# Gabisanth/MaximumAreaCoverageOptimization.jl

Hardware: AMD Instinct MI355X
Metric: MADS objective evals/sec (N UAVs × M fire cells), 1/2/4/8 MI355X (higher is better)
Workload: dtype f64

## Files before the change

maximumareacoverageoptimization.jl_amd/csrc/k_prep.h:

```cpp
#pragma once

#include <hip/hip_runtime.h>
#include <stdint.h>

#include "predicate.h"
#include "k_common.h"

#pragma clang fp contract(off)

namespace mac {


struct PenArgs {
    const double* rmax;
    const double* prev;
    const double* dlimT;
    const double* dlim;
    double tan_half_fov;
};

__device__ __forceinline__ double pen_threshold(const PenArgs& pa, int i)
{
    if (!pa.prev) return 0.0;
    return pa.dlimT ? pa.dlimT[i] : dlim_threshold(pa.dlim[i]);
}

__device__ __forceinline__ double pen_term(double x2, double y2, double R2, int i, int N,
                                           const PenArgs& pa, double T3)
{
    if (pa.prev) {
        const double x1 = pa.prev[i], y1 = pa.prev[N + i], z1 = pa.prev[2 * N + i] / pa.tan_half_fov;
        const double z2 = R2 / pa.tan_half_fov;
        const double ddx = x1 - x2, ddy = y1 - y2, ddz = z1 - z2;
        const double s = ddx * ddx + ddy * ddy + ddz * ddz;
        if (s > T3) return -1.0;
    }
    return pa.rmax ? __builtin_fabs(R2 - pa.rmax[i]) : 0.0;
}

__host__ __device__ __forceinline__ bool diag_rejects(double v, double b, double p, int q,
                                                      double tan_half_fov, double T3)
{
    bool all = true;
#pragma unroll
    for (int sg = 0; sg < 2; ++sg) {
        const double c = sg == 0 ? v + b : v - b;
        double d;
        if (q < 2) {
            d = p - c;
        } else {
            const double z1 = p / tan_half_fov, z2 = c / tan_half_fov;
            d = z1 - z2;
        }
        const double sq = d * d;
        all = all && sq > T3;
    }
    return all;
}


__host__ __device__ __forceinline__ uint64_t splitmix_at(uint64_t state, uint64_t idx)
{
    uint64_t z = state + idx * 0x9E3779B97F4A7C15ull;
    z = (z ^ (z >> 30)) * 0xBF58476D1CE4E5B9ull;
    z = (z ^ (z >> 27)) * 0x94D049BB133111EBull;
    return z ^ (z >> 31);
}

__host__ __device__ __forceinline__ double splitmix_uniform_at(uint64_t state, uint64_t idx)
{
    return (double)(splitmix_at(state, idx) >> 11) * (1.0 / 9007199254740992.0);
}

__host__ __device__ __forceinline__ double ltmads_entry(uint64_t state, int64_t n, int64_t b,
                                                        int64_t r, int64_t c)
{
    if (r < c) return 0.0;
    if (r == c) return (splitmix_uniform_at(state, (uint64_t)r + 1) < 0.5 ? -1.0 : 1.0) * (double)b;
    const int64_t lo = -b + 1, span = 2 * b - 1;
    const double u = splitmix_uniform_at(state, (uint64_t)(n + 1 + r * (r - 1) / 2 + c));
    return (double)(lo + (int64_t)__builtin_floor(u * (double)span));
}

struct MadsState {
    double f;
    int64_t it;
    int ell;
    int skip;
    unsigned long long feas;
    int64_t skipped;
    int64_t succ;
};

struct CandSrc {
    const double* cands;
    int ldc;
    const uint32_t* keysP;
    const float* keysT;
    int ldk;
    const double* xinc;
    const int* rp;
    const int* cp;
    uint64_t state;
    int64_t b;
    int k0;
    const MadsState* mst;
    const int16_t* ltri;
    double delta;
    int route_five;
    __device__ __forceinline__ bool resolve(bool any_poll = false)
    {
        if (!mst) return true;
        const int e = mst->ell;
        if (e < 0 || (!any_poll && mst->skip)) return false;
        b = (int64_t)1 << e;
        return true;
    }
    __device__ __forceinline__ double entry(int n, int r, int c) const
    {
        if (ltri) return r < c ? 0.0 : delta * (double)ltri[(int64_t)r * (r + 1) / 2 + c];
        return ltmads_entry(state, n, b, r, c);
    }
    __device__ __forceinline__ double get(int kl, int v, int N) const
    {
        if (cands) return cands[(int64_t)kl * ldc + v];
        const int n = 3 * N;
        const int k = kl + k0;
        const int kk = k < n ? k : k - n;
        const double d = entry(n, rp[v], cp[kk]);
        return k < n ? xinc[v] + d : xinc[v] - d;
    }
};

#ifndef MAC_PREP_C
#define MAC_PREP_C 8
#endif
constexpr int kPrepC = MAC_PREP_C;
constexpr int kPrepU = 512;

static_assert(kPrepC % 4 == 0 && 32 % kPrepC == 0 && kPrepC <= 64,
              "MAC_PREP_C must divide 32 and be a multiple of 4");
__host__ __device__ inline int keys_ld(int K) { return (K + 31) & ~31; }

struct PrepArgs {
    CandSrc src;
    int N, K;
    PenArgs pa;
    double penalty;
    double* vp;
    int pair;
    int nchain;
    int skip_failed;
    int4* prec;
    Grid g;
    uint32_t* keysP;
    float* keysT;
    int ldk;
    double4* pd;
    uint8_t* dead8;
    MadsState* mst_w;
    unsigned long long* feas;
    int* lreset;
    int xbase;
};

constexpr int kPrepCX = 6;

constexpr uint32_t kKeyEsc = 0x200u << 22;
__device__ __forceinline__ bool key_int(double v, double b, double lim, int& d)
{
    const double f = v - b;
    if (!(f >= -lim && f <= lim)) return false;
    d = (int)f;
    return (double)d == f && __builtin_bit_cast(uint64_t, b + (double)d) == __builtin_bit_cast(uint64_t, v);
}
__device__ __forceinline__ uint32_t key_pack(int dx, int dy, int dr)
{
    return ((uint32_t)dx & 0x7FFu) | (((uint32_t)dy & 0x7FFu) << 11) | (((uint32_t)dr & 0x3FFu) << 22);
}
__device__ __forceinline__ void key_unpack(uint32_t p, float& x, float& y, float& r)
{
    x = (float)((int)(p << 21) >> 21);
    y = (float)((int)(p << 10) >> 21);
    r = (float)((int)p >> 22);
}

__device__ __forceinline__ bool partial_range(double a, double b, double m, double g0, double invS,
                                              int n, int& lo, int& hi)
{
    const double ulo = (a - g0) * invS;
    const double uhi = (b - g0) * invS;
    const double err = (m + __builtin_fabs(g0)) * invS * 1e-14 + 1e-9;
    const double flo = __builtin_floor(ulo - err);
    const double fhi = __builtin_floor(uhi + err);
    if (!(flo == flo) || !(fhi == fhi)) { lo = 0; hi = n - 1; return true; }
    if (fhi < 0.0 || flo > (double)(n - 1)) return false;
    lo = flo < 0.0 ? 0 : (int)flo;
    hi = fhi > (double)(n - 1) ? n - 1 : (int)fhi;
    return true;
}

__host__ __device__ inline int range_shift(int n)
{
    int s = 0;
    while (((n - 1) >> s) > 0xFFFE) ++s;
    return s;
}
__device__ __forceinline__ uint32_t range_pack(bool any, int lo, int hi, int s)
{
    return any ? (uint32_t)(lo >> s) | ((uint32_t)(hi >> s) << 16) : 0xFFFFu;
}
__device__ __forceinline__ void range_unpack(uint32_t lo16, uint32_t hi16, int s, int n, int& lo, int& hi)
{
    lo = (int)(lo16 << s);
    hi = min((int)(((hi16 + 1) << s) - 1), n - 1);
}

#ifdef MAC_DIAG
__device__ uint64_t g_diag_prep[64 * 16];
#define MAC_PREP_STAMP_T(q, t) if (threadIdx.x == (t) && cw < 64 && (q) < 16) g_diag_prep[16 * cw + (q)] = __builtin_amdgcn_s_memrealtime()
#else
#define MAC_PREP_STAMP_T(q, t)
#endif
#define MAC_PREP_STAMP(q) MAC_PREP_STAMP_T(q, 0)

__device__ __forceinline__ void lds_barrier()
{
    asm volatile("s_waitcnt lgkmcnt(0)\n\ts_barrier" ::: "memory");
}

template <int PC>
struct PrepLds {
    double term[PC][kPrepU + 2];
    int wbad[kPrepU / kWave][PC];
    uint32_t wbadm[kPrepU / kWave];
    int wrej[kPrepU / kWave];
    double dred[kPrepU / kWave][4];
};

template <bool kMat, int PC>
__device__ __forceinline__ void prep_block(const PrepArgs& a, int cw, unsigned char* lds)
{
    constexpr int NC = PC;
    PrepLds<NC>& L = *reinterpret_cast<PrepLds<NC>*>(lds);
    auto& term = L.term;
    auto& wbad = L.wbad;
    auto& wbadm = L.wbadm;
    auto& wrej = L.wrej;
    auto& dred = L.dred;
    const int N = a.N, K = a.K;
    const int u = threadIdx.x, lane = u & (kWave - 1), wid = u / kWave;
    const int k0 = cw * PC;
    const int n3 = 3 * N;
    auto cand = [&](int c) { return a.pair ? (c < 4 ? 4 * cw + c : n3 + 4 * cw + c - 4) : k0 + c; };
    const bool obj = a.vp != nullptr;
    const PenArgs& pa = a.pa;
    MAC_PREP_STAMP(0);
    double acc = 0.0;
    bool bad = false;
    const bool excl = obj && pa.prev && (a.prec || a.pd) && a.skip_failed && N <= kPrepU;
    double dmx = -__builtin_inf(), dmy = -__builtin_inf(), dmr = -__builtin_inf();
    double dml = -__builtin_inf();
    uint32_t dead = 0u;
    for (int ib = 0; ib < N; ib += kPrepU) {
        const int nb = min(kPrepU, N - ib);
        const int i = ib + u;
        const bool iv = u < nb;
        const int ii = min(i, N - 1);
        double v[NC][3];
        if (!kMat && PC == 8 && a.pair) {
#pragma unroll
            for (int c = 0; c < 4; ++c) {
                const int col = 4 * cw + c;
#pragma unroll
                for (int q = 0; q < 3; ++q) {
                    const int vv = q * N + ii;
                    const double d = a.src.entry(n3, a.src.rp[vv], a.src.cp[col]);
                    v[c][q] = a.src.xinc[vv] + d;
                    v[c + 4][q] = a.src.xinc[vv] - d;
                }
            }
        } else {
#pragma unroll
            for (int c = 0; c < NC; ++c) {
                const int k = min(cand(c), K - 1);
#pragma unroll
                for (int q = 0; q < 3; ++q) {
                    if constexpr (kMat) v[c][q] = a.src.cands[(int64_t)k * a.src.ldc + q * N + ii];
                    else v[c][q] = a.src.get(k, q * N + ii, N);
                }
            }
        }
        double base[3] = {0.0, 0.0, 0.0};
        if (a.keysP) {
#pragma unroll
            for (int q = 0; q < 3; ++q) {
                if constexpr (kMat) base[q] = a.src.cands[q * N + ii];
                else base[q] = a.src.get(0, q * N + ii, N);
            }
        }
        if (obj) {
            const double x1 = pa.prev ? pa.prev[ii] : 0.0, y1 = pa.prev ? pa.prev[N + ii] : 0.0;
            const double z1 = pa.prev ? pa.prev[2 * N + ii] / pa.tan_half_fov : 0.0;
            const double rm = pa.rmax ? pa.rmax[ii] : 0.0;
            const double T3 = pen_threshold(pa, ii);
            uint32_t wdead = 0u;
#pragma unroll
            for (int c = 0; c < NC; ++c) {
                const double R2 = v[c][2];
                double t = pa.rmax ? __builtin_fabs(R2 - rm) : 0.0;
                if (pa.prev) {
                    const double z2 = R2 / pa.tan_half_fov;
                    const double ddx = x1 - v[c][0], ddy = y1 - v[c][1], ddz = z1 - z2;
                    const double sq = ddx * ddx + ddy * ddy + ddz * ddz;
                    if (sq > T3) t = -1.0;
                }
                term[c][u] = t;
                const uint64_t neg = __ballot(iv && t < 0.0);
                if (lane == 0) wbad[wid][c] = neg != 0;
                wdead |= (neg != 0 ? 1u : 0u) << c;
            }
            if (lane == 0) wbadm[wid] = wdead;
            if (a.mst_w) {
                bool rej = true;
                if (iv) {
                    const double bb = (double)a.src.b;
                    rej = diag_rejects(a.src.xinc[ii], bb, x1, 0, pa.tan_half_fov, T3) &&
                          diag_rejects(a.src.xinc[N + ii], bb, y1, 1, pa.tan_half_fov, T3) &&
                          diag_rejects(a.src.xinc[2 * N + ii], bb, pa.prev[2 * N + ii], 2, pa.tan_half_fov, T3);
                }
                const uint64_t keep = __ballot(!rej);
                if (lane == 0) wrej[wid] = keep == 0;
            }
            MAC_PREP_STAMP(1 + 3 * (ib / kPrepU));
            lds_barrier();
            if (excl) {
                dead = 0u;
#pragma unroll
                for (int w = 0; w < kPrepU / kWave; ++w) dead |= wbadm[w];
                if (a.mst_w) {
                    bool rej = true;
#pragma unroll
                    for (int w = 0; w < kPrepU / kWave; ++w) rej = rej && wrej[w] != 0;
                    if (cw == 0 && u == 0) a.mst_w->skip = rej ? 1 : 0;
                    if (rej) return;
                }
            }
            if (u < NC) {
#pragma unroll
                for (int w = 0; w < kPrepU / kWave; ++w) bad |= wbad[w][u] != 0;
                if (!bad) {
                    __builtin_amdgcn_s_setprio(3);
                    constexpr int kB = 3;
                    const double2* row2 = reinterpret_cast<const double2*>(&term[u][0]);
                    const int nfull = nb / (2 * kB);
                    auto batch = [&](double2 (&buf)[kB], int bt) {
                        const int at = (bt < nfull ? bt : nfull - 1) * kB;
#pragma unroll
                        for (int j = 0; j < kB; ++j) buf[j] = row2[at + j];
                    };
                    auto add = [&](const double2 (&buf)[kB]) {
#pragma unroll
                        for (int j = 0; j < kB; ++j) {
                            acc += buf[j].x;
                            acc += buf[j].y;
                        }
                    };
                    if (nfull > 0) {
                        double2 A[kB], B[kB];
                        batch(A, 0);
#pragma unroll 1
                        for (int bt = 0; bt < nfull; bt += 2) {
                            batch(B, bt + 1);
                            __builtin_amdgcn_sched_barrier(0);
                            add(A);
                            if (bt + 1 >= nfull) break;
                            batch(A, bt + 2);
                            __builtin_amdgcn_sched_barrier(0);
                            add(B);
                        }
                    }
                    for (int q = nfull * 2 * kB; q < nb; ++q) acc += term[u][q];
                    __builtin_amdgcn_s_setprio(0);
                }
            }
            MAC_PREP_STAMP(2 + 3 * (ib / kPrepU));
        }
        if (a.pd && a.keysP && iv) {
#pragma unroll
            for (int c = 0; c < NC; ++c) {
                const double x = v[c][0], y = v[c][1], r = v[c][2];
                if (cand(c) < K && !((dead >> c) & 1u) && r > 0.0 && __builtin_isfinite(x) &&
                    __builtin_isfinite(y)) {
                    double ex = __builtin_fabs(x - base[0]), ey = __builtin_fabs(y - base[1]), er = r - base[2];
                    double el = base[2] - r;
                    if (!(ex <= kDblMax)) ex = __builtin_inf();
                    if (!(ey <= kDblMax)) ey = __builtin_inf();
                    if (!(er == er)) er = __builtin_inf();
                    if (!(el == el)) el = __builtin_inf();
                    dmx = fmax(dmx, ex);
                    dmy = fmax(dmy, ey);
                    dmr = fmax(dmr, er);
                    dml = fmax(dml, el);
                }
            }
        }
        if (a.pd && ib + kPrepU >= N) {
#pragma unroll
            for (int o = 32; o >= 1; o >>= 1) {
                dmx = fmax(dmx, __shfl_xor(dmx, o, kWave));
                dmy = fmax(dmy, __shfl_xor(dmy, o, kWave));
                dmr = fmax(dmr, __shfl_xor(dmr, o, kWave));
                dml = fmax(dml, __shfl_xor(dml, o, kWave));
            }
            if (lane == 0) {
                dred[wid][0] = dmx;
                dred[wid][1] = dmy;
                dred[wid][2] = dmr;
                dred[wid][3] = dml;
            }
        }
        if ((a.prec || a.keysP) && iv) {
            double xa = __builtin_inf(), xb = -__builtin_inf(), ya = __builtin_inf(), yb = -__builtin_inf();
            double xm = 0.0, ym = 0.0, est = 0.0;
            bool any = false;
#pragma unroll
            for (int c = 0; c < NC; ++c) {
                if (!a.prec) break;
                const double x = v[c][0], y = v[c][1], r = v[c][2];
                if (cand(c) < K && !((dead >> c) & 1u) && r > 0.0 && __builtin_isfinite(x) &&
                    __builtin_isfinite(y)) {
                    any = true;
                    xa = fmin(xa, x - r);
                    xb = fmax(xb, x + r);
                    ya = fmin(ya, y - r);
                    yb = fmax(yb, y + r);
                    xm = fmax(xm, __builtin_fabs(x) + r);
                    ym = fmax(ym, __builtin_fabs(y) + r);
                    const double e = 2.0 * r * a.g.invS + 1.0;
                    est += e * e;
                }
            }
            bool kb = false;
            if (a.keysP) {
                uint32_t pk[NC];
#pragma unroll
                for (int c = 0; c < NC; ++c) {
                    int dx = 0, dy = 0, dr = 0;
                    const bool packs = key_int(v[c][0], base[0], 1023.0, dx) &&
                                       key_int(v[c][1], base[1], 1023.0, dy) &&
                                       key_int(v[c][2], base[2], 511.0, dr);
                    pk[c] = packs ? key_pack(dx, dy, dr) : kKeyEsc;
                    if (!packs) {
#pragma unroll
                        for (int q = 0; q < 3; ++q) {
                            const float f = (float)(v[c][q] - base[q]);
                            kb |= !((dead >> c) & 1u) && __builtin_bit_cast(uint64_t, base[q] + (double)f) != __builtin_bit_cast(uint64_t, v[c][q]);
                            a.keysT[(int64_t)(q * N + i) * a.ldk + cand(c)] = f;
                        }
                    }
                }
                uint32_t* const krow = a.keysP + (int64_t)i * a.ldk;
#pragma unroll
                for (int h = 0; h < PC / 4; ++h)
                    *reinterpret_cast<uint4*>(krow + cand(4 * h)) =
                        make_uint4(pk[4 * h], pk[4 * h + 1], pk[4 * h + 2], pk[4 * h + 3]);
            }
            if (a.prec) {
                int x0 = 0, x1 = -1, y0 = 0, y1 = -1;
                any = any && partial_range(xa, xb, xm, a.g.gx0, a.g.invS, a.g.nTx, x0, x1) &&
                      partial_range(ya, yb, ym, a.g.gy0, a.g.invS, a.g.nTy, y0, y1);
                a.prec[(int64_t)cw * N + i] =
                    make_int4((int)range_pack(any, x0, x1, range_shift(a.g.nTx)),
                              (int)range_pack(any, y0, y1, range_shift(a.g.nTy)),
                              __builtin_bit_cast(int, (float)est), kb ? 1 : 0);
            }
        }
        MAC_PREP_STAMP(3 + 3 * (ib / kPrepU));
        if (obj && ib + kPrepU < N) lds_barrier();
    }
    if (obj && u < NC && cand(u) < K) {
        a.vp[cand(u)] = bad ? __builtin_inf() : acc * a.penalty;
        if (a.dead8) a.dead8[cand(u)] = excl && bad ? 1 : 0;
    }
    if (obj && a.feas && wid == 0) {
        const uint64_t ok = __ballot(u < NC && cand(u) < K && !bad);
        if (lane == 0 && ok) atomicAdd(a.feas, (unsigned long long)__popcll(ok));
    }
    if (a.pd) {
        lds_barrier();
        if (u == 0) {
            double4 m = make_double4(dred[0][0], dred[0][1], dred[0][2], dred[0][3]);
            for (int q = 1; q < kPrepU / kWave; ++q) {
                m.x = fmax(m.x, dred[q][0]);
                m.y = fmax(m.y, dred[q][1]);
                m.z = fmax(m.z, dred[q][2]);
                m.w = fmax(m.w, dred[q][3]);
            }
            a.pd[cw] = m;
        }
    }
}

template <bool kGen>
__device__ __forceinline__ void prep_block_x(const PrepArgs& a, int cw, unsigned char* lds)
{
    constexpr int PC = kPrepCX, NC = kGen ? kPrepCX : kPrepCX + 1, NW = kPrepU / kWave;
    PrepLds<kPrepCX + 1>& L = *reinterpret_cast<PrepLds<kPrepCX + 1>*>(lds);
    auto& term = L.term;
    auto& wbad = L.wbad;
    auto& wbadm = L.wbadm;
    auto& wrej = L.wrej;
    auto& dred = L.dred;
    const int N = a.N, K = a.K;
    const int u = threadIdx.x, lane = u & (kWave - 1), wid = u / kWave;
    const bool fw = wid == NW;
    const int k0 = cw * PC;
    const int n3 = 3 * N;
    auto cand = [&](int c) {
        if constexpr (kGen) return c < 3 ? 3 * cw + c : n3 + 3 * cw + c - 3;
        else return c < PC ? k0 + c : a.xbase + cw;
    };
    const bool obj = a.vp != nullptr;
    const PenArgs& pa = a.pa;
    const bool excl = obj && pa.prev && a.skip_failed;
    const bool iv = !fw && u < N;
    const int ii = min(u, N - 1);
    MAC_PREP_STAMP(0);
    double v[NC][3];
    double base[3] = {0.0, 0.0, 0.0};
    if (!fw) {
        if constexpr (kGen) {
#pragma unroll
            for (int q = 0; q < 3; ++q) {
                const int vv = q * N + ii;
                const int rv = a.src.rp[vv];
                const double xv = a.src.xinc[vv];
#pragma unroll
                for (int c = 0; c < 3; ++c) {
                    const double d = a.src.entry(n3, rv, a.src.cp[3 * cw + c]);
                    v[c][q] = xv + d;
                    v[c + 3][q] = xv - d;
                }
                base[q] = xv + a.src.entry(n3, rv, a.src.cp[0]);
            }
        } else {
#pragma unroll
            for (int c = 0; c < NC; ++c) {
                const int k = min(cand(c), K - 1);
#pragma unroll
                for (int q = 0; q < 3; ++q) v[c][q] = a.src.cands[(int64_t)k * a.src.ldc + q * N + ii];
            }
#pragma unroll
            for (int q = 0; q < 3; ++q) base[q] = a.src.cands[q * N + ii];
        }
        if (obj) {
            const double x1 = pa.prev ? pa.prev[ii] : 0.0, y1 = pa.prev ? pa.prev[N + ii] : 0.0;
            const double z1 = pa.prev ? pa.prev[2 * N + ii] / pa.tan_half_fov : 0.0;
            const double rm = pa.rmax ? pa.rmax[ii] : 0.0;
            const double T3 = pen_threshold(pa, ii);
            uint32_t wdead = 0u;
#pragma unroll
            for (int c = 0; c < NC; ++c) {
                const double R2 = v[c][2];
                double t = pa.rmax ? __builtin_fabs(R2 - rm) : 0.0;
                if (pa.prev) {
                    const double z2 = R2 / pa.tan_half_fov;
                    const double ddx = x1 - v[c][0], ddy = y1 - v[c][1], ddz = z1 - z2;
                    const double sq = ddx * ddx + ddy * ddy + ddz * ddz;
                    if (sq > T3) t = -1.0;
                }
                term[c][u] = t;
                const uint64_t neg = __ballot(iv && t < 0.0);
                if (lane == 0) wbad[wid][c] = neg != 0;
                wdead |= (neg != 0 ? 1u : 0u) << c;
            }
            if (lane == 0) wbadm[wid] = wdead;
            if (a.mst_w) {
                bool rej = true;
                if (iv) {
                    const double bb = (double)a.src.b;
                    rej = diag_rejects(a.src.xinc[ii], bb, x1, 0, pa.tan_half_fov, T3) &&
                          diag_rejects(a.src.xinc[N + ii], bb, y1, 1, pa.tan_half_fov, T3) &&
                          diag_rejects(a.src.xinc[2 * N + ii], bb, pa.prev[2 * N + ii], 2, pa.tan_half_fov, T3);
                }
                const uint64_t keep = __ballot(!rej);
                if (lane == 0) wrej[wid] = keep == 0;
            }
        }
    }
    MAC_PREP_STAMP(1);
    uint32_t dead = 0u;
    if (obj) {
        lds_barrier();
        if (excl) {
#pragma unroll
            for (int w = 0; w < NW; ++w) dead |= wbadm[w];
            if (a.mst_w) {
                bool rej = true;
#pragma unroll
                for (int w = 0; w < NW; ++w) rej = rej && wrej[w] != 0;
                if (cw == 0 && u == 0) a.mst_w->skip = rej ? 1 : 0;
                if (rej) return;
            }
        }
    }
    MAC_PREP_STAMP(2);
    if (fw) {
        bool bad = false;
        double acc = 0.0;
        if (obj && lane < NC) {
#pragma unroll
            for (int w = 0; w < NW; ++w) bad |= wbad[w][lane] != 0;
            if (!bad) {
                constexpr int kB = 6;
                const double2* row2 = reinterpret_cast<const double2*>(&term[lane][0]);
                const int nfull = N / (2 * kB);
                __builtin_amdgcn_s_setprio(3);
                auto batch = [&](double2 (&buf)[kB], int bt) {
                    const int at = (bt < nfull ? bt : nfull - 1) * kB;
#pragma unroll
                    for (int j = 0; j < kB; ++j) buf[j] = row2[at + j];
                };
                auto add = [&](const double2 (&buf)[kB]) {
#pragma unroll
                    for (int j = 0; j < kB; ++j) {
                        acc += buf[j].x;
                        acc += buf[j].y;
                    }
                };
                if (nfull > 0) {
                    double2 A[kB], B[kB];
                    batch(A, 0);
#pragma unroll 1
                    for (int bt = 0; bt < nfull; bt += 2) {
                        batch(B, bt + 1);
                        __builtin_amdgcn_sched_barrier(0);
                        add(A);
                        if (bt + 1 >= nfull) break;
                        batch(A, bt + 2);
                        __builtin_amdgcn_sched_barrier(0);
                        add(B);
                    }
                }
                for (int q = nfull * 2 * kB; q < N; ++q) acc += term[lane][q];
                __builtin_amdgcn_s_setprio(0);
            }
            MAC_PREP_STAMP_T(3, kPrepU);
            if (cand(lane) < K) {
                a.vp[cand(lane)] = bad ? __builtin_inf() : acc * a.penalty;
                if (a.dead8) a.dead8[cand(lane)] = excl && bad ? 1 : 0;
            }
        }
        if (obj && a.feas) {
            const uint64_t ok = __ballot(lane < NC && cand(lane) < K && !bad);
            if (lane == 0 && ok) atomicAdd(a.feas, (unsigned long long)__popcll(ok));
        }
    } else {
        double dmx = -__builtin_inf(), dmy = -__builtin_inf(), dmr = -__builtin_inf(), dml = -__builtin_inf();
        uint32_t pk[NC];
        bool kb = false;
#pragma unroll
        for (int c = 0; c < NC; ++c) {
            const double x = v[c][0], y = v[c][1], r = v[c][2];
            int dx = 0, dy = 0, dr = 0;
            const bool packs = key_int(x, base[0], 1023.0, dx) && key_int(y, base[1], 1023.0, dy) &&
                               key_int(r, base[2], 511.0, dr);
            pk[c] = packs ? key_pack(dx, dy, dr) : kKeyEsc;
            if (!packs && iv && cand(c) < K) {
#pragma unroll
                for (int q = 0; q < 3; ++q) {
                    const float f = (float)(v[c][q] - base[q]);
                    if constexpr (kGen)
                        kb |= !((dead >> c) & 1u) &&
                              __builtin_bit_cast(uint64_t, base[q] + (double)f) != __builtin_bit_cast(uint64_t, v[c][q]);
                    a.keysT[(int64_t)(q * N + u) * a.ldk + cand(c)] = f;
                }
            }
            if (a.pd && iv && cand(c) < K && !((dead >> c) & 1u) && r > 0.0 && __builtin_isfinite(x) &&
                __builtin_isfinite(y)) {
                double ex = __builtin_fabs(x - base[0]), ey = __builtin_fabs(y - base[1]), er = r - base[2];
                double el = base[2] - r;
                if (!(ex <= kDblMax)) ex = __builtin_inf();
                if (!(ey <= kDblMax)) ey = __builtin_inf();
                if (!(er == er)) er = __builtin_inf();
                if (!(el == el)) el = __builtin_inf();
                dmx = fmax(dmx, ex);
                dmy = fmax(dmy, ey);
                dmr = fmax(dmr, er);
                dml = fmax(dml, el);
            }
        }
        if (iv) {
            uint32_t* const krow = a.keysP + (int64_t)u * a.ldk;
            if constexpr (kGen) {
#pragma unroll
                for (int c = 0; c < NC; ++c) krow[cand(c)] = pk[c];
            } else {
                static_assert(PC % 2 == 0, "an even candidate count");
#pragma unroll
                for (int h = 0; h < PC / 2; ++h)
                    *reinterpret_cast<uint2*>(krow + k0 + 2 * h) = make_uint2(pk[2 * h], pk[2 * h + 1]);
                if (cand(PC) < K) krow[cand(PC)] = pk[PC];
            }
        }
        if (kGen && a.prec && iv) {
            double xa = __builtin_inf(), xb = -__builtin_inf(), ya = __builtin_inf(), yb = -__builtin_inf();
            double xm = 0.0, ym = 0.0, est = 0.0;
            bool any = false;
#pragma unroll
            for (int c = 0; c < NC; ++c) {
                const double x = v[c][0], y = v[c][1], r = v[c][2];
                if (cand(c) < K && !((dead >> c) & 1u) && r > 0.0 && __builtin_isfinite(x) &&
                    __builtin_isfinite(y)) {
                    any = true;
                    xa = fmin(xa, x - r);
                    xb = fmax(xb, x + r);
                    ya = fmin(ya, y - r);
                    yb = fmax(yb, y + r);
                    xm = fmax(xm, __builtin_fabs(x) + r);
                    ym = fmax(ym, __builtin_fabs(y) + r);
                    const double e = 2.0 * r * a.g.invS + 1.0;
                    est += e * e;
                }
            }
            int x0 = 0, x1 = -1, y0 = 0, y1 = -1;
            any = any && partial_range(xa, xb, xm, a.g.gx0, a.g.invS, a.g.nTx, x0, x1) &&
                  partial_range(ya, yb, ym, a.g.gy0, a.g.invS, a.g.nTy, y0, y1);
            a.prec[(int64_t)cw * N + u] =
                make_int4((int)range_pack(any, x0, x1, range_shift(a.g.nTx)),
                          (int)range_pack(any, y0, y1, range_shift(a.g.nTy)),
                          __builtin_bit_cast(int, (float)est), kb ? 1 : 0);
        }
        if (a.pd) {
#pragma unroll
            for (int o = 32; o >= 1; o >>= 1) {
                dmx = fmax(dmx, __shfl_xor(dmx, o, kWave));
                dmy = fmax(dmy, __shfl_xor(dmy, o, kWave));
                dmr = fmax(dmr, __shfl_xor(dmr, o, kWave));
                dml = fmax(dml, __shfl_xor(dml, o, kWave));
            }
            if (lane == 0) {
                dred[wid][0] = dmx;
                dred[wid][1] = dmy;
                dred[wid][2] = dmr;
                dred[wid][3] = dml;
            }
        }
    }
    if (a.pd) {
        lds_barrier();
        if (u == 0) {
            double4 m = make_double4(dred[0][0], dred[0][1], dred[0][2], dred[0][3]);
            for (int q = 1; q < NW; ++q) {
                m.x = fmax(m.x, dred[q][0]);
                m.y = fmax(m.y, dred[q][1]);
                m.z = fmax(m.z, dred[q][2]);
                m.w = fmax(m.w, dred[q][3]);
            }
            a.pd[cw] = m;
        }
    }
}

template <int PC, bool kX = false, bool kGen = false>
__device__ __forceinline__ void prep_body(uint64_t* ts, PrepArgs& a)
{
    ts_begin(ts);
    if (a.lreset && blockIdx.x == 0 && threadIdx.x == 0) *a.lreset = 0;
    if (!a.src.resolve(true)) {
        ts_end(ts);
        return;
    }
    const int per = (int)((gridDim.x + 7) / 8), b = (int)blockIdx.x;
    const int cw = (int)(gridDim.x % 8) == 0 ? (b % 8) * per + b / 8 : b;
    __shared__ __attribute__((aligned(16))) unsigned char lds[sizeof(PrepLds<kX ? PC + 1 : PC>)];
    if constexpr (kX) {
        prep_block_x<kGen>(a, cw, lds);
    } else if (a.src.cands) {
        prep_block<true, PC>(a, cw, lds);
    } else {
        prep_block<false, PC>(a, cw, lds);
    }
    ts_end(ts);
}

__global__ __launch_bounds__(kPrepU) __attribute__((amdgpu_waves_per_eu(4))) void prep_kernel(uint64_t* ts, PrepArgs a)
{
    prep_body<kPrepC>(ts, a);
}

template <bool kGen>
__global__ __launch_bounds__(kPrepU + kWave) __attribute__((amdgpu_waves_per_eu(6))) void prep_x_kernel(uint64_t* ts, PrepArgs a)
{
    prep_body<kPrepCX, true, kGen>(ts, a);
}

__global__ void disk_prep_kernel(CandSrc src, int N, int K, DiskRec* __restrict__ disks)
{
    const int64_t t = (int64_t)blockIdx.x * blockDim.x + threadIdx.x;
    if (t >= (int64_t)N * K) return;
    const int k = (int)(t / N), i = (int)(t % N);
    disks[t] = make_disk(src.get(k, i, N), src.get(k, N + i, N), src.get(k, 2 * N + i, N));
}

}
```

Before: 44.17 million.

## Overlap penalty fold and key packing with feasibility checks in prep kernel

Restructures the prep kernel's non-generated path so the rmax penalty terms are written to LDS before the distance check. The fold warp can then sum them while worker warps do the feasibility test and key packing, with global loads ordered by sched_barriers to issue the radius loads first. Key packing for the candidate path now runs before the barrier that waits on failure flags, so packing overlaps the synchronization. In exchange the fold runs even for candidates later marked bad, an extra barrier is added, and the control flow is more complex.

```diff
diff --git a/maximumareacoverageoptimization.jl_amd/csrc/k_prep.h b/maximumareacoverageoptimization.jl_amd/csrc/k_prep.h
--- a/maximumareacoverageoptimization.jl_amd/csrc/k_prep.h
+++ b/maximumareacoverageoptimization.jl_amd/csrc/k_prep.h
@@ -219,8 +219,10 @@
 #ifdef MAC_DIAG
 __device__ uint64_t g_diag_prep[64 * 16];
 #define MAC_PREP_STAMP_T(q, t) if (threadIdx.x == (t) && cw < 64 && (q) < 16) g_diag_prep[16 * cw + (q)] = __builtin_amdgcn_s_memrealtime()
+#define MAC_PREP_STAMP_XY(q) do { asm volatile("s_waitcnt vmcnt(0)" ::: "memory"); MAC_PREP_STAMP_T(q, 0); } while (0)
 #else
 #define MAC_PREP_STAMP_T(q, t)
+#define MAC_PREP_STAMP_XY(q)
 #endif
 #define MAC_PREP_STAMP(q) MAC_PREP_STAMP_T(q, 0)
 
@@ -527,9 +529,84 @@
     const bool iv = !fw && u < N;
     const int ii = min(u, N - 1);
     MAC_PREP_STAMP(0);
-    double v[NC][3];
-    double base[3] = {0.0, 0.0, 0.0};
-    if (!fw) {
+    auto failures = [&](uint32_t& dead) {
+        if (!excl) return false;
+#pragma unroll
+        for (int w = 0; w < NW; ++w) dead |= wbadm[w];
+        if (!a.mst_w) return false;
+        bool rej = true;
+#pragma unroll
+        for (int w = 0; w < NW; ++w) rej = rej && wrej[w] != 0;
+        if (cw == 0 && u == 0) a.mst_w->skip = rej ? 1 : 0;
+        return rej;
+    };
+    auto fold = [&](double& acc) {
+        constexpr int kB = 6;
+        const double2* row2 = reinterpret_cast<const double2*>(&term[lane][0]);
+        const int nfull = N / (2 * kB);
+        __builtin_amdgcn_s_setprio(3);
+        auto batch = [&](double2 (&buf)[kB], int bt) {
+            const int at = (bt < nfull ? bt : nfull - 1) * kB;
+#pragma unroll
+            for (int j = 0; j < kB; ++j) buf[j] = row2[at + j];
+        };
+        auto add = [&](const double2 (&buf)[kB]) {
+#pragma unroll
+            for (int j = 0; j < kB; ++j) {
+                acc += buf[j].x;
+                acc += buf[j].y;
+            }
+        };
+        if (nfull > 0) {
+            double2 A[kB], B[kB];
+            batch(A, 0);
+#pragma unroll 1
+            for (int bt = 0; bt < nfull; bt += 2) {
+                batch(B, bt + 1);
+                __builtin_amdgcn_sched_barrier(0);
+                add(A);
+                if (bt + 1 >= nfull) break;
+                batch(A, bt + 2);
+                __builtin_amdgcn_sched_barrier(0);
+                add(B);
+            }
+        }
+        for (int q = nfull * 2 * kB; q < N; ++q) acc += term[lane][q];
+        __builtin_amdgcn_s_setprio(0);
+    };
+    if (fw) {
+        bool bad = false;
+        double acc = 0.0;
+        if (obj) {
+            const bool mine = lane < NC && cand(lane) < K;
+            if constexpr (!kGen) {
+                lds_barrier();
+                if (mine) fold(acc);
+                MAC_PREP_STAMP_T(3, kPrepU);
+            }
+            lds_barrier();
+            uint32_t dead = 0u;
+            if (failures(dead)) return;
+            if (mine) {
+#pragma unroll
+                for (int w = 0; w < NW; ++w) bad |= wbad[w][lane] != 0;
+                if constexpr (kGen) {
+                    if (!bad) fold(acc);
+                    MAC_PREP_STAMP_T(3, kPrepU);
+                }
+                a.vp[cand(lane)] = bad ? __builtin_inf() : acc * a.penalty;
+                if (a.dead8) a.dead8[cand(lane)] = excl && bad ? 1 : 0;
+            }
+            if (a.feas) {
+                const uint64_t ok = __ballot(mine && !bad);
+                if (lane == 0 && ok) atomicAdd(a.feas, (unsigned long long)__popcll(ok));
+            }
+        }
+    } else {
+        double v[NC][3];
+        double base[3] = {0.0, 0.0, 0.0};
+        double rm = 0.0;
+        double x1 = 0.0, y1 = 0.0, p1 = 0.0, dl = 0.0;
         if constexpr (kGen) {
 #pragma unroll
             for (int q = 0; q < 3; ++q) {
@@ -544,21 +621,46 @@
                 }
                 base[q] = xv + a.src.entry(n3, rv, a.src.cp[0]);
             }
+            if (obj) {
+                if (pa.rmax) rm = pa.rmax[ii];
+                if (pa.prev) {
+                    x1 = pa.prev[ii], y1 = pa.prev[N + ii], p1 = pa.prev[2 * N + ii];
+                    dl = pa.dlimT ? pa.dlimT[ii] : pa.dlim[ii];
+                }
+            }
         } else {
-#pragma unroll
-            for (int c = 0; c < NC; ++c) {
-                const int k = min(cand(c), K - 1);
-#pragma unroll
-                for (int q = 0; q < 3; ++q) v[c][q] = a.src.cands[(int64_t)k * a.src.ldc + q * N + ii];
-            }
+            const double* cp[NC];
+#pragma unroll
+            for (int c = 0; c < NC; ++c) cp[c] = a.src.cands + (int64_t)min(cand(c), K - 1) * a.src.ldc + ii;
+#pragma unroll
+            for (int c = 0; c < NC; ++c) v[c][2] = cp[c][2 * N];
+            const double* const anyp = a.src.cands + ii;
+            rm = *(obj && pa.rmax ? pa.rmax + ii : anyp);
+            __builtin_amdgcn_sched_barrier(0);
 #pragma unroll
             for (int q = 0; q < 3; ++q) base[q] = a.src.cands[q * N + ii];
+            const bool c3 = obj && pa.prev;
+            x1 = *(c3 ? pa.prev + ii : anyp), y1 = *(c3 ? pa.prev + N + ii : anyp);
+            p1 = *(c3 ? pa.prev + 2 * N + ii : anyp);
+            dl = *(!c3 ? anyp : pa.dlimT ? pa.dlimT + ii : pa.dlim + ii);
+            __builtin_amdgcn_sched_barrier(0);
+#pragma unroll
+            for (int c = 0; c < NC; ++c) {
+                v[c][0] = cp[c][0];
+                v[c][1] = cp[c][N];
+                __builtin_amdgcn_sched_barrier(0);
+            }
+            if (obj) {
+#pragma unroll
+                for (int c = 0; c < NC; ++c) term[c][u] = pa.rmax ? __builtin_fabs(v[c][2] - rm) : 0.0;
+                MAC_PREP_STAMP(1);
+                lds_barrier();
+                MAC_PREP_STAMP(2);
+            }
         }
         if (obj) {
-            const double x1 = pa.prev ? pa.prev[ii] : 0.0, y1 = pa.prev ? pa.prev[N + ii] : 0.0;
-            const double z1 = pa.prev ? pa.prev[2 * N + ii] / pa.tan_half_fov : 0.0;
-            const double rm = pa.rmax ? pa.rmax[ii] : 0.0;
-            const double T3 = pen_threshold(pa, ii);
+            const double z1 = pa.prev ? p1 / pa.tan_half_fov : 0.0;
+            const double T3 = !pa.prev ? 0.0 : pa.dlimT ? dl : dlim_threshold(dl);
             uint32_t wdead = 0u;
 #pragma unroll
             for (int c = 0; c < NC; ++c) {
@@ -570,7 +672,7 @@
                     const double sq = ddx * ddx + ddy * ddy + ddz * ddz;
                     if (sq > T3) t = -1.0;
                 }
-                term[c][u] = t;
+                if constexpr (kGen) term[c][u] = t;
                 const uint64_t neg = __ballot(iv && t < 0.0);
                 if (lane == 0) wbad[wid][c] = neg != 0;
                 wdead |= (neg != 0 ? 1u : 0u) << c;
@@ -582,101 +684,64 @@
                     const double bb = (double)a.src.b;
                     rej = diag_rejects(a.src.xinc[ii], bb, x1, 0, pa.tan_half_fov, T3) &&
                           diag_rejects(a.src.xinc[N + ii], bb, y1, 1, pa.tan_half_fov, T3) &&
-                          diag_rejects(a.src.xinc[2 * N + ii], bb, pa.prev[2 * N + ii], 2, pa.tan_half_fov, T3);
+                          diag_rejects(a.src.xinc[2 * N + ii], bb, p1, 2, pa.tan_half_fov, T3);
                 }
                 const uint64_t keep = __ballot(!rej);
                 if (lane == 0) wrej[wid] = keep == 0;
             }
         }
-    }
-    MAC_PREP_STAMP(1);
-    uint32_t dead = 0u;
-    if (obj) {
-        lds_barrier();
-        if (excl) {
-#pragma unroll
-            for (int w = 0; w < NW; ++w) dead |= wbadm[w];
-            if (a.mst_w) {
-                bool rej = true;
-#pragma unroll
-                for (int w = 0; w < NW; ++w) rej = rej && wrej[w] != 0;
-                if (cw == 0 && u == 0) a.mst_w->skip = rej ? 1 : 0;
-                if (rej) return;
-            }
-        }
-    }
-    MAC_PREP_STAMP(2);
-    if (fw) {
-        bool bad = false;
-        double acc = 0.0;
-        if (obj && lane < NC) {
-#pragma unroll
-            for (int w = 0; w < NW; ++w) bad |= wbad[w][lane] != 0;
-            if (!bad) {
-                constexpr int kB = 6;
-                const double2* row2 = reinterpret_cast<const double2*>(&term[lane][0]);
-                const int nfull = N / (2 * kB);
-                __builtin_amdgcn_s_setprio(3);
-                auto batch = [&](double2 (&buf)[kB], int bt) {
-                    const int at = (bt < nfull ? bt : nfull - 1) * kB;
-#pragma unroll
-                    for (int j = 0; j < kB; ++j) buf[j] = row2[at + j];
-                };
-                auto add = [&](const double2 (&buf)[kB]) {
-#pragma unroll
-                    for (int j = 0; j < kB; ++j) {
-                        acc += buf[j].x;
-                        acc += buf[j].y;
-                    }
-                };
-                if (nfull > 0) {
-                    double2 A[kB], B[kB];
-                    batch(A, 0);
-#pragma unroll 1
-                    for (int bt = 0; bt < nfull; bt += 2) {
-                        batch(B, bt + 1);
-                        __builtin_amdgcn_sched_barrier(0);
-                        add(A);
-                        if (bt + 1 >= nfull) break;
-                        batch(A, bt + 2);
-                        __builtin_amdgcn_sched_barrier(0);
-                        add(B);
-                    }
-                }
-                for (int q = nfull * 2 * kB; q < N; ++q) acc += term[lane][q];
-                __builtin_amdgcn_s_setprio(0);
-            }
-            MAC_PREP_STAMP_T(3, kPrepU);
-            if (cand(lane) < K) {
-                a.vp[cand(lane)] = bad ? __builtin_inf() : acc * a.penalty;
-                if (a.dead8) a.dead8[cand(lane)] = excl && bad ? 1 : 0;
-            }
-        }
-        if (obj && a.feas) {
-            const uint64_t ok = __ballot(lane < NC && cand(lane) < K && !bad);
-            if (lane == 0 && ok) atomicAdd(a.feas, (unsigned long long)__popcll(ok));
-        }
-    } else {
+        uint32_t dead = 0u;
+        bool kb = false;
+        auto escape = [&](int c) {
+            if (!(iv && cand(c) < K)) return;
+#pragma unroll
+            for (int q = 0; q < 3; ++q) {
+                const float f = (float)(v[c][q] - base[q]);
+                if constexpr (kGen)
+                    kb |= !((dead >> c) & 1u) &&
+                          __builtin_bit_cast(uint64_t, base[q] + (double)f) != __builtin_bit_cast(uint64_t, v[c][q]);
+                a.keysT[(int64_t)(q * N + u) * a.ldk + cand(c)] = f;
+            }
+        };
+        auto keys = [&]() {
+            uint32_t pk[NC];
+#pragma unroll
+            for (int c = 0; c < NC; ++c) {
+                int dr = 0;
+                pk[c] = key_int(v[c][2], base[2], 511.0, dr) ? key_pack(0, 0, dr) : kKeyEsc;
+            }
+#pragma unroll
+            for (int c = 0; c < NC; ++c) {
+                int dx = 0, dy = 0;
+                const bool packs = pk[c] != kKeyEsc && key_int(v[c][0], base[0], 1023.0, dx) &&
+                                   key_int(v[c][1], base[1], 1023.0, dy);
+                pk[c] = packs ? pk[c] | key_pack(dx, dy, 0) : kKeyEsc;
+                if (!packs) escape(c);
+            }
+            if (iv) {
+                uint32_t* const krow = a.keysP + (int64_t)u * a.ldk;
+                static_assert(PC % 2 == 0, "an even candidate count");
+#pragma unroll
+                for (int h = 0; h < PC / 2; ++h)
+                    *reinterpret_cast<uint2*>(krow + k0 + 2 * h) = make_uint2(pk[2 * h], pk[2 * h + 1]);
+                if constexpr (NC > PC)
+                    if (cand(PC) < K) krow[cand(PC)] = pk[PC];
+            }
+        };
+        if constexpr (kGen) {
+            MAC_PREP_STAMP(1);
+        } else {
+            MAC_PREP_STAMP_XY(4);
+            keys();
+            MAC_PREP_STAMP(5);
+        }
+        if (obj) {
+            lds_barrier();
+            if (failures(dead)) return;
+        }
         double dmx = -__builtin_inf(), dmy = -__builtin_inf(), dmr = -__builtin_inf(), dml = -__builtin_inf();
-        uint32_t pk[NC];
-        bool kb = false;
-#pragma unroll
-        for (int c = 0; c < NC; ++c) {
+        auto bound = [&](int c) {
             const double x = v[c][0], y = v[c][1], r = v[c][2];
-            int dx = 0, dy = 0, dr = 0;
-            const bool packs = key_int(x, base[0], 1023.0, dx) && key_int(y, base[1], 1023.0, dy) &&
-                               key_int(r, base[2], 511.0, dr);
-            pk[c] = packs ? key_pack(dx, dy, dr) : kKeyEsc;
-            if (!packs && iv && cand(c) < K) {
-#pragma unroll
-                for (int q = 0; q < 3; ++q) {
-                    const float f = (float)(v[c][q] - base[q]);
-                    if constexpr (kGen)
-                        kb |= !((dead >> c) & 1u) &&
-                              __builtin_bit_cast(uint64_t, base[q] + (double)f) != __builtin_bit_cast(uint64_t, v[c][q]);
-                    a.keysT[(int64_t)(q * N + u) * a.ldk + cand(c)] = f;
-                }
-            }
             if (a.pd && iv && cand(c) < K && !((dead >> c) & 1u) && r > 0.0 && __builtin_isfinite(x) &&
                 __builtin_isfinite(y)) {
                 double ex = __builtin_fabs(x - base[0]), ey = __builtin_fabs(y - base[1]), er = r - base[2];
@@ -690,19 +755,28 @@
                 dmr = fmax(dmr, er);
                 dml = fmax(dml, el);
             }
-        }
-        if (iv) {
-            uint32_t* const krow = a.keysP + (int64_t)u * a.ldk;
-            if constexpr (kGen) {
+        };
+        if constexpr (kGen) {
+            MAC_PREP_STAMP(2);
+            uint32_t pk[NC];
+#pragma unroll
+            for (int c = 0; c < NC; ++c) {
+                int dx = 0, dy = 0, dr = 0;
+                const bool packs = key_int(v[c][0], base[0], 1023.0, dx) && key_int(v[c][1], base[1], 1023.0, dy) &&
+                                   key_int(v[c][2], base[2], 511.0, dr);
+                pk[c] = packs ? key_pack(dx, dy, dr) : kKeyEsc;
+                if (!packs) escape(c);
+                bound(c);
+            }
+            if (iv) {
+                uint32_t* const krow = a.keysP + (int64_t)u * a.ldk;
 #pragma unroll
                 for (int c = 0; c < NC; ++c) krow[cand(c)] = pk[c];
-            } else {
-                static_assert(PC % 2 == 0, "an even candidate count");
-#pragma unroll
-                for (int h = 0; h < PC / 2; ++h)
-                    *reinterpret_cast<uint2*>(krow + k0 + 2 * h) = make_uint2(pk[2 * h], pk[2 * h + 1]);
-                if (cand(PC) < K) krow[cand(PC)] = pk[PC];
-            }
+            }
+        } else {
+            MAC_PREP_STAMP(6);
+#pragma unroll
+            for (int c = 0; c < NC; ++c) bound(c);
         }
         if (kGen && a.prec && iv) {
             double xa = __builtin_inf(), xb = -__builtin_inf(), ya = __builtin_inf(), yb = -__builtin_inf();
```

Measured after the change: 42.60 million. -3.6%, worse.
